# dakom/awsm-renderer

Hardware: AMD Instinct MI355X
Metric: frames/sec + shaded Mpix/s, 4K Sponza glTF, 1/2/4/8 MI355X (higher is better)
Workload: dtype f32; 1 GPU; Sponza-class procedural atrium (configs[3]): 262144 triangles, 25 materials, 69 textures, 3840x2160, geometry pass + opaque pass, single-sample, MipmapMode::None; triangles=262144, width=3840, height=2160, draws=92, frame_overlap=True, stream_handoff=device flags (k_handoff_signal / k_handoff_wait), camera=orbit, one turn per 240 frames, environment=uniform cubes (builder default), opaque_route=lean (k_shade_lean + k_shade_todo), library=awsm-renderer_amd/libawsm_hip.so

## Files before the change

### awsm-renderer_amd/csrc/device_math.hpp

```cpp
#pragma once
#include <hip/hip_runtime.h>
#include <hip/hip_fp16.h>
#include <stdint.h>

namespace awsm {

struct f2 { float x, y; };
struct f3 { float x, y, z; };
struct f4 { float x, y, z, w; };
struct m4 { f4 c[4]; };
struct m3 { f3 c[3]; };

#define AWSM_DI __device__ __forceinline__

constexpr float kPi = 3.1415926535897932384626433832795f;
constexpr float kTau = 6.283185307179586476925286766559f;
constexpr float kEps = 1e-4f;

AWSM_DI f2 mk2(float x, float y) { return {x, y}; }
AWSM_DI f3 mk3(float x, float y, float z) { return {x, y, z}; }
AWSM_DI f4 mk4(float x, float y, float z, float w) { return {x, y, z, w}; }
AWSM_DI f3 splat3(float s) { return {s, s, s}; }
AWSM_DI f3 operator+(f3 a, f3 b) { return {a.x + b.x, a.y + b.y, a.z + b.z}; }
AWSM_DI f3 operator-(f3 a, f3 b) { return {a.x - b.x, a.y - b.y, a.z - b.z}; }
AWSM_DI f3 operator*(f3 a, f3 b) { return {a.x * b.x, a.y * b.y, a.z * b.z}; }
AWSM_DI f3 operator*(f3 a, float s) { return {a.x * s, a.y * s, a.z * s}; }
AWSM_DI f3 operator/(f3 a, float s) { return {a.x / s, a.y / s, a.z / s}; }
AWSM_DI f3 operator-(f3 a) { return {-a.x, -a.y, -a.z}; }
AWSM_DI float dot(f3 a, f3 b) { return (a.x * b.x + a.y * b.y) + a.z * b.z; }
AWSM_DI f3 cross(f3 a, f3 b) { return {a.y * b.z - a.z * b.y, a.z * b.x - a.x * b.z, a.x * b.y - a.y * b.x}; }
AWSM_DI float length(f3 a) { return sqrtf(dot(a, a)); }
AWSM_DI f3 normalize(f3 a) { const float inv = 1.0f / length(a); return {a.x * inv, a.y * inv, a.z * inv}; }
AWSM_DI float mixf(float a, float b, float t) { return a * (1.0f - t) + b * t; }
AWSM_DI f3 mix3(f3 a, f3 b, float t) { float s = 1.0f - t; return {a.x * s + b.x * t, a.y * s + b.y * t, a.z * s + b.z * t}; }
AWSM_DI f3 min3(f3 a, f3 b) { return {fminf(a.x, b.x), fminf(a.y, b.y), fminf(a.z, b.z)}; }
AWSM_DI float clampf(float x, float lo, float hi) { return fminf(fmaxf(x, lo), hi); }
AWSM_DI float saturate(float x) { return clampf(x, 0.0f, 1.0f); }
AWSM_DI float inverse_sqrt(float x) { return 1.0f / sqrtf(x); }
AWSM_DI float signf(float x) { return x > 0.0f ? 1.0f : (x < 0.0f ? -1.0f : 0.0f); }

AWSM_DI f4 mul(const m4& m, f4 v) {
    f4 r;
    r.x = ((m.c[0].x * v.x + m.c[1].x * v.y) + m.c[2].x * v.z) + m.c[3].x * v.w;
    r.y = ((m.c[0].y * v.x + m.c[1].y * v.y) + m.c[2].y * v.z) + m.c[3].y * v.w;
    r.z = ((m.c[0].z * v.x + m.c[1].z * v.y) + m.c[2].z * v.z) + m.c[3].z * v.w;
    r.w = ((m.c[0].w * v.x + m.c[1].w * v.y) + m.c[2].w * v.z) + m.c[3].w * v.w;
    return r;
}
AWSM_DI f3 mul(const m3& m, f3 v) {
    f3 r;
    r.x = (m.c[0].x * v.x + m.c[1].x * v.y) + m.c[2].x * v.z;
    r.y = (m.c[0].y * v.x + m.c[1].y * v.y) + m.c[2].y * v.z;
    r.z = (m.c[0].z * v.x + m.c[1].z * v.y) + m.c[2].z * v.z;
    return r;
}
AWSM_DI m3 upper3(const m4& m) {
    m3 r;
    r.c[0] = {m.c[0].x, m.c[0].y, m.c[0].z};
    r.c[1] = {m.c[1].x, m.c[1].y, m.c[1].z};
    r.c[2] = {m.c[2].x, m.c[2].y, m.c[2].z};
    return r;
}
AWSM_DI m4 load_m4(const float* p) {
    const float4* q = reinterpret_cast<const float4*>(p);
    m4 m;
#pragma unroll
    for (int i = 0; i < 4; i++) { float4 v = q[i]; m.c[i] = {v.x, v.y, v.z, v.w}; }
    return m;
}

AWSM_DI float round_f16(float x) { return __half2float(__float2half_rn(x)); }
AWSM_DI unsigned short f16_bits(float x) { return __half_as_ushort(__float2half_rn(x)); }
AWSM_DI float f16_bits_to_f32(unsigned short h) { return __half2float(__ushort_as_half(h)); }

AWSM_DI float det_atan2f(float y, float x) {
    float ax = fabsf(x), ay = fabsf(y);
    float mx = fmaxf(ax, ay), mn = fminf(ax, ay);
    if (mx == 0.0f) return 0.0f;
    float a = mn / mx;
    float s = a * a;
    float r = 0.0027856871f;
    r = r * s - 0.0158660002f;
    r = r * s + 0.0424557589f;
    r = r * s - 0.0749753043f;
    r = r * s + 0.106448799f;
    r = r * s - 0.142070308f;
    r = r * s + 0.199934542f;
    r = r * s - 0.333331466f;
    r = r * s;
    r = r * a + a;
    if (ay > ax) r = 1.57079637f - r;
    if (x < 0.0f) r = 3.14159274f - r;
    if (y < 0.0f) r = -r;
    return r;
}

AWSM_DI f3 safe_normalize(f3 n) {
    float len_sq = dot(n, n);
    if (len_sq > 0.0f) return n * inverse_sqrt(len_sq);
    return {0.0f, 0.0f, 1.0f};
}
AWSM_DI float inverse_square(float range, float dist) {
    if (range == 0.0f) return 1.0f / fmaxf(dist * dist, 0.01f);
    float denom = dist * dist + 1.0f;
    float falloff = 1.0f - (dist * dist) / (range * range);
    return saturate(falloff * falloff) / denom;
}
AWSM_DI f2 encode_octahedral(f3 n_in) {
    const float inv = 1.0f / ((fabsf(n_in.x) + fabsf(n_in.y)) + fabsf(n_in.z));
    f3 n = {n_in.x * inv, n_in.y * inv, n_in.z * inv};
    if (n.z < 0.0f) {
        float wx = (1.0f - fabsf(n.y)) * signf(n.x);
        float wy = (1.0f - fabsf(n.x)) * signf(n.y);
        n.x = wx; n.y = wy;
    }
    return {n.x * 0.5f + 0.5f, n.y * 0.5f + 0.5f};
}
AWSM_DI f3 decode_octahedral(f2 e) {
    float fx = e.x * 2.0f - 1.0f, fy = e.y * 2.0f - 1.0f;
    f3 n = {fx, fy, (1.0f - fabsf(fx)) - fabsf(fy)};
    float t = clampf(-n.z, 0.0f, 1.0f);
    float vx = (n.x >= 0.0f) ? -t : t;
    float vy = (n.y >= 0.0f) ? -t : t;
    n = {n.x + vx, n.y + vy, n.z};
    return normalize(n);
}
struct TB { f3 t, b; };
AWSM_DI TB canonical_tb(f3 n) {
    TB r;
    if (n.z < -0.9999999f) {
        r.t = {0.0f, -1.0f, 0.0f};
        r.b = {-1.0f, 0.0f, 0.0f};
    } else {
        float a = 1.0f / (1.0f + n.z);
        float bb = (-n.x * n.y) * a;
        r.t = {1.0f - (n.x * n.x) * a, bb, -n.x};
        r.b = {bb, 1.0f - (n.y * n.y) * a, -n.y};
    }
    return r;
}
AWSM_DI f4 pack_normal_tangent(f3 N, f3 T, float s) {
    f2 oct = encode_octahedral(N);
    TB tb = canonical_tb(N);
    float x = dot(T, tb.t);
    float y = dot(T, tb.b);
    float theta = det_atan2f(y, x);
    float angle_u = (theta + kPi) / kTau;
    float sign_u = (s > 0.0f) ? 1.0f : 0.0f;
    return {oct.x, oct.y, angle_u, sign_u};
}
struct TBN { f3 N, T, B; };
AWSM_DI TBN unpack_normal_tangent(f4 rgba) {
    TBN r;
    r.N = decode_octahedral({rgba.x, rgba.y});
    float theta = rgba.z * kTau - kPi;
    float s = (rgba.w >= 0.5f) ? 1.0f : -1.0f;
    TB tb0 = canonical_tb(r.N);
    float c = cosf(theta), sn = sinf(theta);
    r.T = normalize(tb0.t * c + tb0.b * sn);
    r.B = normalize(cross(r.N, r.T)) * s;
    return r;
}

AWSM_DI float interp3_strict(float b0, float b1, float b2, float x0, float x1, float x2) { return (b0 * x0 + b1 * x1) + b2 * x2; }
AWSM_DI float affine2_strict(float a, float b, float c, float x, float y) { return (a * x + b * y) + c; }

AWSM_DI float blend_over_f16(float src, float dst, float one_minus_a) { return round_f16(src + dst * one_minus_a); }
AWSM_DI float resolve4_f16(float s0, float s1, float s2, float s3) { return round_f16((((s0 + s1) + s2) + s3) * 0.25f); }

}
```

### awsm-renderer_amd/csrc/kernels_shade.hip

```cpp
#include <type_traits>
#include "frame_params.hpp"
#include "raster_setup.hpp"

#ifndef AWSM_LEAN_WAVES
#define AWSM_LEAN_WAVES 6
#endif

namespace awsm {

struct GBufferTexel {
    f4 packed_nt;
    float bx, by;
    f4 bary_derivs;
};
template <bool DERIVS>
AWSM_DI GBufferTexel reconstruct_core(const TriSetup& t, float4 n0, float4 n1, float4 n2, float4 t0, float4 t1, float4 t2, int cx, int cy) {
    GBufferTexel g;
    g.bary_derivs = {0.0f, 0.0f, 0.0f, 0.0f};
    const double Xc = sample_coord((cx << 8) + 128), Yc = sample_coord((cy << 8) + 128);
    const EdgeVals ev = tri_edges_d(t, Xc, Yc);
    const float e0 = (float)ev.E[0] * t.iw[0], e1 = (float)ev.E[1] * t.iw[1], e2 = (float)ev.E[2] * t.iw[2];
    const float inv_esum = 1.0f / ((e0 + e1) + e2);
    const float b0 = e0 * inv_esum, b1 = e1 * inv_esum, b2 = e2 * inv_esum;
    const f3 Ni = {(b0 * n0.x + b1 * n1.x) + b2 * n2.x, (b0 * n0.y + b1 * n1.y) + b2 * n2.y, (b0 * n0.z + b1 * n1.z) + b2 * n2.z};
    const f4 Ti = {(b0 * t0.x + b1 * t1.x) + b2 * t2.x, (b0 * t0.y + b1 * t1.y) + b2 * t2.y,
                   (b0 * t0.z + b1 * t1.z) + b2 * t2.z, (b0 * t0.w + b1 * t1.w) + b2 * t2.w};
    const f4 p = pack_normal_tangent(normalize(Ni), normalize(mk3(Ti.x, Ti.y, Ti.z)), Ti.w);
    g.packed_nt = {round_f16(p.x), round_f16(p.y), round_f16(p.z), round_f16(p.w)};
    g.bx = round_f16(b0);
    g.by = round_f16(b1);
    if (DERIVS) {
        const EdgeVals eh = tri_edges_d(t, sample_coord(((cx ^ 1) << 8) + 128), Yc), evv = tri_edges_d(t, Xc, sample_coord(((cy ^ 1) << 8) + 128));
        const float h0 = (float)eh.E[0] * t.iw[0], h1 = (float)eh.E[1] * t.iw[1], h2 = (float)eh.E[2] * t.iw[2];
        const float w0 = (float)evv.E[0] * t.iw[0], w1 = (float)evv.E[1] * t.iw[1], w2 = (float)evv.E[2] * t.iw[2];
        const float ish = 1.0f / ((h0 + h1) + h2), isv = 1.0f / ((w0 + w1) + w2);
        const float hb0 = h0 * ish, hb1 = h1 * ish, vb0 = w0 * isv, vb1 = w1 * isv;
        const float ddx0 = (cx & 1) ? b0 - hb0 : hb0 - b0, ddx1 = (cx & 1) ? b1 - hb1 : hb1 - b1;
        const float ddy0 = (cy & 1) ? b0 - vb0 : vb0 - b0, ddy1 = (cy & 1) ? b1 - vb1 : vb1 - b1;
        g.bary_derivs = {round_f16(ddx0), round_f16(ddy0), round_f16(ddx1), round_f16(ddy1)};
    }
    return g;
}
template <bool DERIVS>
AWSM_DI GBufferTexel reconstruct_gbuffer(const FrameDev& f, uint32_t rank, int cx, int cy) {
    TriSetup t;
    tri_rec_load(f.tri_rec + rank, t);
    const float4 n0 = f.nrm[(size_t)rank * 3], n1 = f.nrm[(size_t)rank * 3 + 1], n2 = f.nrm[(size_t)rank * 3 + 2];
    const float4 t0 = f.tan[(size_t)rank * 3], t1 = f.tan[(size_t)rank * 3 + 1], t2 = f.tan[(size_t)rank * 3 + 2];
    return reconstruct_core<DERIVS>(t, n0, n1, n2, t0, t1, t2, cx, cy);
}

AWSM_DI f2 strict_oct_of(const FrameDev& f, uint32_t rank, int cx, int cy) {
    TriSetup t;
    tri_rec_load(f.tri_rec + rank, t);
    const float4 n0 = f.nrm[(size_t)rank * 3], n1 = f.nrm[(size_t)rank * 3 + 1], n2 = f.nrm[(size_t)rank * 3 + 2];
    const double Xc = sample_coord((cx << 8) + 128), Yc = sample_coord((cy << 8) + 128);
    const EdgeVals ev = tri_edges_d(t, Xc, Yc);
    const float e0 = (float)ev.E[0] * t.iw[0], e1 = (float)ev.E[1] * t.iw[1], e2 = (float)ev.E[2] * t.iw[2];
    const float inv_esum = 1.0f / ((e0 + e1) + e2);
    const float b0 = e0 * inv_esum, b1 = e1 * inv_esum, b2 = e2 * inv_esum;
    const f3 Ni = {(b0 * n0.x + b1 * n1.x) + b2 * n2.x, (b0 * n0.y + b1 * n1.y) + b2 * n2.y, (b0 * n0.z + b1 * n1.z) + b2 * n2.z};
    const f2 oct = encode_octahedral(normalize(Ni));
    return mk2(round_f16(oct.x), round_f16(oct.y));
}
AWSM_DI f3 strict_normal_of(const FrameDev& f, uint32_t rank, int cx, int cy) { return decode_octahedral(strict_oct_of(f, rank, cx, cy)); }
AWSM_DI uint32_t oct_word(f2 oct) { return (uint32_t)f16_bits(oct.x) | ((uint32_t)f16_bits(oct.y) << 16); }
AWSM_DI f2 oct_of_word(uint32_t w) { return mk2(__half2float(__ushort_as_half((unsigned short)(w & 0xFFFFu))), __half2float(__ushort_as_half((unsigned short)(w >> 16)))); }

AWSM_DI bool row_owned(const FrameDev& f, int py) {
    if (py < (int)f.sy0 || py >= (int)f.sy1) return false;
    return f.band_n <= 1u || (((uint32_t)py >> kTileShift) % f.band_n) == f.band_r;
}

constexpr float kEdgeNormalThreshold = 0.95f, kEdgeDepthThreshold = 0.02f, kEdgeMsaaDepthThreshold = 0.02f;
AWSM_DI float view_space_depth(const m4& inv_proj, float depth, float px, float py, float W, float H) {
    if (inv_proj.c[0].z == 0.0f && inv_proj.c[1].z == 0.0f && inv_proj.c[0].w == 0.0f && inv_proj.c[1].w == 0.0f)
        return (inv_proj.c[2].z * depth + inv_proj.c[3].z) / (inv_proj.c[2].w * depth + inv_proj.c[3].w);
    const f4 view_pos = mul(inv_proj, mk4((px / W) * 2.0f - 1.0f, 1.0f - (py / H) * 2.0f, depth, 1.0f));
    return view_pos.z / view_pos.w;
}
AWSM_DI float key_depth(unsigned long long k) { return k == ~0ull ? 1.0f : __uint_as_float((uint32_t)(k >> 32)); }
AWSM_DI uint32_t key_rank(unsigned long long k) { return 0xFFFFFFFFu - (uint32_t)(k & 0xFFFFFFFFull); }
AWSM_DI bool edge_mask_depth_msaa(const m4& inv_proj, const unsigned long long k4[4], float pcx, float pcy, float W, float H) {
    uint32_t count = 0; float dmin = 1e9f, dmax = -1e9f;
#pragma unroll
// ... 1780 lines not shown
                const m4 inv_proj = cload_m4(f.camera, 256u);
                const unsigned long long k4[4] = {((unsigned long long)ka.y << 32) | ka.x, ((unsigned long long)ka.w << 32) | ka.z, ((unsigned long long)kb.y << 32) | kb.x, ((unsigned long long)kb.w << 32) | kb.z};
                sure = edge_mask_depth_msaa_filtered(inv_proj, k4, (float)cx + 0.5f, (float)cy + 0.5f, (float)f.width, (float)f.height);
                test = !sure;
            }
        }
        const unsigned long long m_sure = __builtin_amdgcn_ballot_w64(sure), m_test = __builtin_amdgcn_ballot_w64(test);
        if (lane == 0u) *reinterpret_cast<ulonglong2*>(f.msaa_edge_bits + (size_t)(b.blk * 4u + (tid >> 6)) * 2u) = make_ulonglong2(m_sure, m_test);
        want_c0 = sure || test;
    }
    bool hud = false;
    if (!ITEMS && !MSAA && f.hud_vis && inside) { const u32x2 hk = gload<u32x2>(f.hud_vis, pv << 3); hud = (hk.x & hk.y) != 0xFFFFFFFFu; }
    if (hud) { store_pixel(f, p, f4{0.0f, 0.0f, 0.0f, 0.0f}); key = {0xFFFFFFFFu, 0xFFFFFFFFu}; }
    const bool hit = inside && (key.x & key.y) != 0xFFFFFFFFu;
    if (!ITEMS && inside && !hit && !hud) {
        const f4 sky = skybox_color(sc, f, cx, cy);
        store_pixel(f, p, sky);
        if (MSAA) {
            f.msaa_cells[pv] = make_uint2(0u, 0xFFFFFFFFu);
            if (want_c0) f.msaa_color0[pv] = make_float4(sky.x, sky.y, sky.z, sky.w);
        }
    }
    unsigned long long rem = __builtin_amdgcn_ballot_w64(hit);
    if (rem == 0ull) return true;
    const uint32_t rank = hit ? ~key.x : 0xFFFFFFFFu;
    const float depth = __uint_as_float(key.y);

    asm volatile("; MARK level1");
    unsigned long long src_base; uint32_t src_stride;
    {
        const uint32_t j = lane;
        const unsigned long long rec = (unsigned long long)f.tri_rec, nr = (unsigned long long)f.nrm, tn = (unsigned long long)f.tan, tsh = (unsigned long long)f.tri_shade;
        src_base = j < 5u ? rec + j * 16u : (j < 8u ? nr + (j - 5u) * 16u : (j < 11u ? tn + (j - 8u) * 16u : tsh + (j - 11u) * 16u));
        src_stride = j < 5u ? (uint32_t)kTriRecBytes : (j < 11u ? 48u : 32u);
    }
    uint32_t my_slot = kLeanNone, n_slots = 0u;
    while (rem != 0ull && n_slots < kLeanSlots) {
        const uint32_t r = (uint32_t)__builtin_amdgcn_readlane((int)rank, (int)__builtin_ctzll(rem));
        if (rank == r) my_slot = n_slots;
        if (lane < kLeanChunks)
            __builtin_amdgcn_global_load_lds((const AWSM_AS1 void*)(src_base + (unsigned long long)r * src_stride), (AWSM_AS3 void*)&st->q[n_slots][0], 16, 0, 0);
        rem &= ~__builtin_amdgcn_uicmp(rank, r, 32 );
        n_slots++;
    }
    asm volatile("s_waitcnt vmcnt(0)" ::: "memory");
    const bool staged = my_slot != kLeanNone;
    const uint4* rec = &st->q[staged ? my_slot : 0u][0];
    uint4 ts0 = rec[11], ts1 = rec[12];
    TriRecRaw raw;
    raw.q0 = bits_float4(rec[0]); raw.q1 = bits_float4(rec[1]); raw.q2 = bits_float4(rec[2]); raw.d3 = bits_double2(rec[3]); raw.d4 = bits_double2(rec[4]);
    float4 n0 = bits_float4(rec[5]), n1 = bits_float4(rec[6]), n2 = bits_float4(rec[7]);
    float4 t0 = bits_float4(rec[8]), t1 = bits_float4(rec[9]), t2 = bits_float4(rec[10]);
    if (hit && !staged) {
        ts0 = as_uint4(gload<u32x4>(f.tri_shade, rank << 5)); ts1 = as_uint4(gload<u32x4>(f.tri_shade, (rank << 5) + 16u));
        const uint32_t ro = rank * (uint32_t)kTriRecBytes, vo = rank * 48u;
        raw.q0 = as_float4(gload<f32x4>(f.tri_rec, ro)); raw.q1 = as_float4(gload<f32x4>(f.tri_rec, ro + 16u)); raw.q2 = as_float4(gload<f32x4>(f.tri_rec, ro + 32u));
        { const f64x2 a = gload<f64x2>(f.tri_rec, ro + 48u), c = gload<f64x2>(f.tri_rec, ro + 64u); raw.d3 = make_double2(a.x, a.y); raw.d4 = make_double2(c.x, c.y); }
        n0 = as_float4(gload<f32x4>(f.nrm, vo)); n1 = as_float4(gload<f32x4>(f.nrm, vo + 16u)); n2 = as_float4(gload<f32x4>(f.nrm, vo + 32u));
        t0 = as_float4(gload<f32x4>(f.tan, vo)); t1 = as_float4(gload<f32x4>(f.tan, vo + 16u)); t2 = as_float4(gload<f32x4>(f.tan, vo + 32u));
    }

    asm volatile("; MARK strict");
    TriSetup t;
    tri_rec_unpack(raw, t);
    const GBufferTexel g = reconstruct_core<(GRAD != 0)>(t, n0, n1, n2, t0, t1, t2, cx, cy);
    if (MSAA && hit) f.msaa_cells[pv] = make_uint2(oct_word(mk2(g.packed_nt.x, g.packed_nt.y)), key.y);
    const float bz = (1.0f - g.bx) - g.by;
    float u = interp3_strict(g.bx, g.by, bz, __uint_as_float(ts0.z), __uint_as_float(ts1.x), __uint_as_float(ts1.z));
    float v = interp3_strict(g.bx, g.by, bz, __uint_as_float(ts0.w), __uint_as_float(ts1.y), __uint_as_float(ts1.w));
    const uint32_t draw = ts0.x & 0x00FFFFFFu;
    const uint32_t d0 = (uint32_t)__builtin_amdgcn_readlane((int)draw, (int)__builtin_ctzll(__builtin_amdgcn_ballot_w64(hit)));
    const bool one_draw = __builtin_amdgcn_ballot_w64(hit && draw != d0) == 0ull;
    f2 ddx = {0.0f, 0.0f}, ddy = {0.0f, 0.0f};
    float m2 = 0.0f;
    float r2min = 0.0f; f2 major = {0.0f, 0.0f};
    if (GRAD) {
        const float x0 = __uint_as_float(ts0.z), y0 = __uint_as_float(ts0.w), x1 = __uint_as_float(ts1.x), y1 = __uint_as_float(ts1.y), x2 = __uint_as_float(ts1.z), y2 = __uint_as_float(ts1.w);
        const float dAlphaDx = g.bary_derivs.x, dAlphaDy = g.bary_derivs.y, dBetaDx = g.bary_derivs.z, dBetaDy = g.bary_derivs.w;
        const float dGammaDx = -dAlphaDx - dBetaDx, dGammaDy = -dAlphaDy - dBetaDy;
        ddx = {x0 * dAlphaDx + x1 * dBetaDx + x2 * dGammaDx, y0 * dAlphaDx + y1 * dBetaDx + y2 * dGammaDx};
        ddy = {x0 * dAlphaDy + x1 * dBetaDy + x2 * dGammaDy, y0 * dAlphaDy + y1 * dBetaDy + y2 * dGammaDy};
        const bool tiny = (fabsf(dAlphaDx) + fabsf(dAlphaDy) + fabsf(dBetaDx) + fabsf(dBetaDy)) < 1e-20f;
        const bool ok = (ddx.x == ddx.x) && (ddx.y == ddx.y) && (ddy.x == ddy.x) && (ddy.y == ddy.y);
        if (tiny || !ok) { ddx = {0.0f, 0.0f}; ddy = {0.0f, 0.0f}; }
    }
    if (GRAD == 0) {
    } else if (one_draw) {
        const uint32_t lo = d0 * (uint32_t)sizeof(LeanDrawDev);
        if (cload<uint32_t>(f.draw_lean, lo) & 8u) {
            const f32x4 ta = cload<f32x4>(f.draw_lean, lo + 176u); const f32x2a4 tb = cload<f32x2a4>(f.draw_lean, lo + 192u);
            const float u2 = affine2_strict(ta.x, ta.y, tb.x, u, v), v2 = affine2_strict(ta.z, ta.w, tb.y, u, v);
            u = u2; v = v2;
            if (GRAD) { ddx = {ta.x * ddx.x + ta.y * ddx.y, ta.z * ddx.x + ta.w * ddx.y}; ddy = {ta.x * ddy.x + ta.y * ddy.y, ta.z * ddy.x + ta.w * ddy.y}; }
        }
    } else {
// ... 17 lines not shown
    f3 base, emissive;
    float metallic_in, roughness_in, normal_scale, occlusion_strength, normal_bias, occlusion_bias;
    uint32_t exists;
    lean::Tap tp0, tp1, tp2, tp3, tp4;
    lean::TapG tg0, tg1, tg2, tg3, tg4;
    constexpr uint32_t kNeed = GRAD == 2 ? 7u : (GRAD ? 3u : 1u);
    auto fetch_all = [&](float uu, float vv, float m2e, bool act, const uint32_t tex_mask = 31u, const bool factors = true) {
        if (one_draw) {
            const uint32_t lo = d0 * (uint32_t)sizeof(LeanDrawDev);
            const u32x4 L0 = cload<u32x4>(f.draw_lean, lo), L1 = cload<u32x4>(f.draw_lean, lo + 16u), L2 = cload<u32x4>(f.draw_lean, lo + 32u);
            const u32x4 L3 = cload<u32x4>(f.draw_lean, lo + 48u), L4 = cload<u32x4>(f.draw_lean, lo + 64u);
            const u32x2 L5 = cload<u32x2>(f.draw_lean, lo + 80u), L5s = cload<u32x2>(f.draw_lean, lo + 88u);
            if (GRAD == 0) {
                if (L0.x & 8u) {
                    const f32x4 ta = cload<f32x4>(f.draw_lean, lo + 176u); const f32x2a4 tb = cload<f32x2a4>(f.draw_lean, lo + 192u);
                    const float u2 = affine2_strict(ta.x, ta.y, tb.x, uu, vv), v2 = affine2_strict(ta.z, ta.w, tb.y, uu, vv);
                    uu = u2; vv = v2;
                }
                todo = todo || __builtin_amdgcn_ballot_w64(hit && !(fabsf(uu) <= 32768.0f && fabsf(vv) <= 32768.0f)) != 0ull;
            }
            todo = todo || (L0.x & kNeed) != kNeed;
            const uint32_t exs = todo ? 0u : L0.x >> 8;
            const uint32_t ex = act ? exs & tex_mask : 0u;
            if (GRAD) {
                const u32x4 G0 = cload<u32x4>(f.draw_lean, lo + 96u), G1 = cload<u32x4>(f.draw_lean, lo + 112u), G2 = cload<u32x4>(f.draw_lean, lo + 128u);
                const u32x4 G3 = cload<u32x4>(f.draw_lean, lo + 144u), G4 = cload<u32x4>(f.draw_lean, lo + 160u);
                if (ex & 1u) lean::fetch_trilinear(lean::decode_g(G0.x, G0.y, G0.z, G0.w), m2e, uu, vv, tg0);
                if (ex & 2u) lean::fetch_trilinear(lean::decode_g(G1.x, G1.y, G1.z, G1.w), m2e, uu, vv, tg1);
                if (ex & 4u) lean::fetch_trilinear(lean::decode_g(G2.x, G2.y, G2.z, G2.w), m2e, uu, vv, tg2);
                if (ex & 8u) lean::fetch_trilinear(lean::decode_g(G3.x, G3.y, G3.z, G3.w), m2e, uu, vv, tg3);
                if (ex & 16u) lean::fetch_trilinear(lean::decode_g(G4.x, G4.y, G4.z, G4.w), m2e, uu, vv, tg4);
            } else {
                if (ex & 1u) lean::fetch_s(lean::decode_s(L3.x, L3.y), uu, vv, tp0);
                if (ex & 2u) lean::fetch_s(lean::decode_s(L3.z, L3.w), uu, vv, tp1);
                if (ex & 4u) lean::fetch_s(lean::decode_s(L4.x, L4.y), uu, vv, tp2);
                if (ex & 8u) lean::fetch_s(lean::decode_s(L4.z, L4.w), uu, vv, tp3);
                if (ex & 16u) lean::fetch_s(lean::decode_s(L5.x, L5.y), uu, vv, tp4);
            }
            exists = exs;
            if (factors) {
            metallic_in = __uint_as_float(L0.y); roughness_in = __uint_as_float(L0.z); normal_scale = __uint_as_float(L0.w);
            base = {__uint_as_float(L1.x), __uint_as_float(L1.y), __uint_as_float(L1.z)}; occlusion_strength = __uint_as_float(L1.w);
            emissive = {__uint_as_float(L2.x), __uint_as_float(L2.y), __uint_as_float(L2.z)}; normal_bias = __uint_as_float(L2.w); occlusion_bias = __uint_as_float(L5s.x);
            }
        } else {
            const uint32_t lo = draw * (uint32_t)sizeof(LeanDrawDev);
// ... 52 lines not shown
    auto mid = [&]() {
    asm volatile("; MARK standard");
    const float pxf = (float)cx, pyf = (float)cy;
    const float* M = f.pix2view;
    const float hx = M[0] * pxf + (M[4] * pyf + (M[8] * depth + M[12])), hy = M[1] * pxf + (M[5] * pyf + (M[9] * depth + M[13]));
    const float hz = M[2] * pxf + (M[6] * pyf + (M[10] * depth + M[14])), hw = M[3] * pxf + (M[7] * pyf + (M[11] * depth + M[15]));
    const float ivw = fm::rcp(fmaxf(hw, 1e-8f));
    const f3 vp = {hx * ivw, hy * ivw, hz * ivw};
    const float* R = f.view_rot;
    const f3 rel = {R[0] * vp.x + (R[3] * vp.y + R[6] * vp.z), R[1] * vp.x + (R[4] * vp.y + R[7] * vp.z), R[2] * vp.x + (R[5] * vp.y + R[8] * vp.z)};
    world_position = {rel.x + f.cam_pos[0], rel.y + f.cam_pos[1], rel.z + f.cam_pos[2]};
#ifdef AWSM_STRICT_POSITION
    world_position = strict_world_position(cload_m4(f.camera, 256u), cload_m4(f.camera, 320u), cx, cy, (float)f.width, (float)f.height, depth);
#endif
    if (f.cam_ortho) {
        surface_to_camera = mk3(f.ortho_view_dir[0], f.ortho_view_dir[1], f.ortho_view_dir[2]);
    } else {
        const f3 to_camera = mk3(f.cam_pos[0], f.cam_pos[1], f.cam_pos[2]) - world_position;
        surface_to_camera = fm::fdot(to_camera, to_camera) > 0.0f ? fm::fsafe_normalize(to_camera) : mk3(0.0f, 0.0f, 1.0f);
    }
    asm volatile("; MARK tbn");
    tbn = fm::funpack_normal_tangent(g.packed_nt);
    normal = tbn.N;
    };
    bool shared_fp = false;
    float Lm = 0.0f;
    auto lean_word = [&](auto one, uint32_t off) {
        if constexpr (decltype(one)::value) return cload<uint32_t>(f.draw_lean, d0 * (uint32_t)sizeof(LeanDrawDev) + off);
        else return gload<uint32_t>(f.draw_lean, draw * (uint32_t)sizeof(LeanDrawDev) + off);
    };
    auto lean_quad = [&](auto one, uint32_t off) {
        if constexpr (decltype(one)::value) return cload<u32x4>(f.draw_lean, d0 * (uint32_t)sizeof(LeanDrawDev) + off);
        else return gload<u32x4>(f.draw_lean, draw * (uint32_t)sizeof(LeanDrawDev) + off);
    };
    auto decide = [&](auto one) {
        const uint32_t fl = lean_word(one, 0u);
        const uint32_t exs = (fl & kNeed) == kNeed ? (fl >> 8) & 31u : 0u;
        int lw_min = 15, top_min = 15;
#pragma unroll
        for (uint32_t k = 0; k < (uint32_t)kCoreTextures; k++) {
            const uint32_t w1 = lean_word(one, 96u + 16u * k + 4u);
            const int lw = (int)(w1 >> 24), lv = (int)((w1 >> 16) & 15u);
            if (exs & (1u << k)) { lw_min = min(lw_min, lw); top_min = min(top_min, lv - 1 - lw); }
        }
        Lm = 0.5f * __builtin_amdgcn_logf(fmaxf(m2c, 1e-30f));
        const bool in = exs != 0u && Lm > -(float)lw_min && Lm < (float)top_min;
// ... 192 lines not shown
    for (uint32_t i = 0; i < n_lights; i++) {
        const f32x4 pre0 = cload<f32x4>(f.lights_pre, i * 32u), pre1 = cload<f32x4>(f.lights_pre, i * 32u + 16u);
        const uint32_t kind = (uint32_t)pre0.w;
        f3 light_dir = {pre0.x, pre0.y, pre0.z}, radiance = {pre1.x, pre1.y, pre1.z};
        if (kind == 2u || kind == 3u) {
            const f32x4 pos_range = cload<f32x4>(lights, i * 64u);
            const f3 stl = mk3(pos_range.x, pos_range.y, pos_range.z) - world_position;
            const float d2 = fm::fdot(stl, stl);
            const float inv_d = d2 > 0.0f ? fm::rsq(d2) : 0.0f;
            const float dist = d2 * inv_d;
            float att;
            if (pos_range.w == 0.0f) att = fm::rcp(fmaxf(dist * dist, 0.01f));
            else { const float fo = 1.0f - fm::fdiv(dist * dist, pos_range.w * pos_range.w); att = fm::fdiv(saturate(fo * fo), dist * dist + 1.0f); }
            const f3 to_light = stl * inv_d;
            if (kind == 3u) {
                const f32x4 dir_inner = cload<f32x4>(lights, i * 64u + 16u), kind_outer = cload<f32x4>(lights, i * 64u + 48u);
                const float cos_l = fm::fdot(to_light, -light_dir);
                const float sm = saturate(fm::fdiv(cos_l - kind_outer.y, dir_inner.w - kind_outer.y));
                att = att * (sm * sm);
            }
            light_dir = to_light;
            radiance = radiance * att;
#ifndef AWSM_NO_LIGHT_SKIP
            if (__builtin_amdgcn_ballot_w64(!(att == 0.0f)) == 0ull) continue;
#endif
        } else if (kind != 1u) { light_dir = {0.0f, 0.0f, 0.0f}; radiance = {0.0f, 0.0f, 0.0f}; }
        lean::direct(lit, light_dir, radiance, color);
    }
    asm volatile("; MARK store");
    if (ITEMS) { item->color = color; return true; }
    store_pixel(f, p, {color.x, color.y, color.z, 1.0f});
    if (MSAA && want_c0) f.msaa_color0[pv] = make_float4(color.x, color.y, color.z, 1.0f);
    return true;
}
template <int GRAD, bool MSAA>
AWSM_DI void lean_block(const DevScene* __restrict__ sc, const FrameDev& f, const ShadeBlock& b, const uint32_t wg, const uint32_t tid, LeanStage* __restrict__ st) {
    (void)lean_core<GRAD, MSAA, false>(sc, f, b, wg, tid, st, nullptr);
}
#ifndef AWSM_ANISO_WAVES
#define AWSM_ANISO_WAVES 4
#endif
#ifndef AWSM_LEAN_COUNTERS
#define AWSM_LEAN_COUNTERS 8
#endif
constexpr uint32_t kLeanCounters = AWSM_LEAN_COUNTERS;
#ifndef AWSM_LEAN_GRAD_WAVES
#define AWSM_LEAN_GRAD_WAVES 5
#endif
template <bool PERSIST, int GRAD, bool MSAA>
// ... 11 lines not shown
    const uint32_t w = __builtin_amdgcn_readfirstlane((blockIdx.x >> 3) * 4u + (threadIdx.x >> 6));
    uint32_t zero;
    asm volatile("v_mov_b32 %0, 0" : "=v"(zero));
    uint32_t c = w % kLeanCounters, tried = 0u;
    uint32_t* ctr0 = f.lean_next + (xcd * kLeanCounters) * 16u + zero;
    uint32_t nxt = 0u;
    if (PERSIST && lane == 0u) nxt = atomicAdd(ctr0 + c * 16u, 1u);
    for (uint32_t j = w;;) {
        if (PERSIST) {
            j = __builtin_amdgcn_readfirstlane(nxt) * kLeanCounters + c;
            while (j >= share && ++tried < kLeanCounters) {
                c = (c + 1u) % kLeanCounters;
                if (lane == 0u) nxt = atomicAdd(ctr0 + c * 16u, 1u);
                j = __builtin_amdgcn_readfirstlane(nxt) * kLeanCounters + c;
            }
            if (j >= share) break;
            if (lane == 0u) nxt = atomicAdd(ctr0 + c * 16u, 1u);
        }
        const uint32_t kb = j >> 2, bcol = kb & ((1u << lp) - 1u), brow = (kb >> lp) * 8u + xcd;
        if (bcol < bx_n && j < share) {
            ShadeBlock b;
            shade_block_at(f, b, brow, bcol);
            lean_block<GRAD, MSAA>(sc, f, b, ((kb >> lp) * bx_n + bcol) * 8u + xcd, ((j & 3u) << 6) | lane, st);
        }
        if (!PERSIST) break;
    }
}

constexpr uint32_t kEdgeRecBytes = 260;
struct NeighbourCell { float nx, ny, nz; uint32_t depth_bits; uint32_t state; };

AWSM_DI void publish_cell(NeighbourCell* cells, int lx, int ly, const FrameDev& f, int px, int py) {
    NeighbourCell c = {0.0f, 0.0f, 0.0f, 0u, 0u};
    if (px >= 0 && px < (int)f.width && py >= (int)f.y0 && py < (int)f.y1) {
        unsigned long long k;
        if (f.band_n > 1u && (((uint32_t)py >> kTileShift) % f.band_n) != f.band_r) {
            const uint32_t ty = (uint32_t)py >> kTileShift, which = ((uint32_t)py & (uint32_t)(kTile - 1)) == 0u ? 0u : 1u;
            k = f.msaa_halo ? f.msaa_halo[((((size_t)(ty % f.band_n) * f.halo_bands + ty / f.band_n) * 2u + which) * f.width) + (size_t)px] : ~0ull;
        } else k = f.vis[((size_t)py * f.width + (size_t)px) * 4];
        c.state = 1u;
        if (k != ~0ull) {
            const f3 n = strict_normal_of(f, key_rank(k), px, py);
            c.nx = n.x; c.ny = n.y; c.nz = n.z; c.depth_bits = (uint32_t)(k >> 32); c.state = 2u;
        }
    }
    cells[(ly + 1) * 18 + (lx + 1)] = c;
}
// ... 403 lines not shown
    const DrawDev dr = draws[tri_info[rank] & 0x00FFFFFFu];
    const uint32_t material_meta_offset = *reinterpret_cast<const uint32_t*>(sc->buf[AWSM_BUF_GEOM_META] + dr.geom_meta_off + 36);
    const uint32_t* mm = reinterpret_cast<const uint32_t*>(sc->buf[AWSM_BUF_MATERIAL_META] + (size_t)(material_meta_offset / 256u) * 256u);
    out[0] = 1u; out[1] = mm[0]; out[2] = mm[1]; out[3] = rank - dr.first_tri;
}

__global__ void k_rgba16f_to_rg16f(const uint16_t* __restrict__ in, uint32_t* __restrict__ out, uint32_t n) {
    const uint32_t i = blockIdx.x * 256u + threadIdx.x;
    if (i < n) out[i] = (uint32_t)in[(size_t)i * 4] | ((uint32_t)in[(size_t)i * 4 + 1] << 16);
}

}

extern "C" void awsm_launch_resolve_draws(const awsm::DevScene* sc, const awsm::FrameDev* f, hipStream_t s) {
    if (f->n_draws) hipLaunchKernelGGL(awsm::k_resolve_draws, dim3((8u * f->n_draws + 255u) / 256u), dim3(256), 0, s, sc, *f);
}
#define AWSM_LAUNCH_G(g, K, grid, block, ...) do { if ((g) == 2) hipLaunchKernelGGL((K<2>), grid, block, 0, s, __VA_ARGS__); else if ((g) == 1) hipLaunchKernelGGL((K<1>), grid, block, 0, s, __VA_ARGS__); \
                                                   else hipLaunchKernelGGL((K<0>), grid, block, 0, s, __VA_ARGS__); } while (0)
#define AWSM_LAUNCH_G2(g, K, B, grid, block, ...) do { if ((g) == 2) hipLaunchKernelGGL((K<2, B>), grid, block, 0, s, __VA_ARGS__); else if ((g) == 1) hipLaunchKernelGGL((K<1, B>), grid, block, 0, s, __VA_ARGS__); \
                                                       else hipLaunchKernelGGL((K<0, B>), grid, block, 0, s, __VA_ARGS__); } while (0)
#define AWSM_LAUNCH_SG(g, K, S, grid, block, ...) do { if ((g) == 2) hipLaunchKernelGGL((K<S, 2>), grid, block, 0, s, __VA_ARGS__); else if ((g) == 1) hipLaunchKernelGGL((K<S, 1>), grid, block, 0, s, __VA_ARGS__); \
                                                       else hipLaunchKernelGGL((K<S, 0>), grid, block, 0, s, __VA_ARGS__); } while (0)
static inline int mip_mode(const awsm::FrameDev* f) { return f->mipmap ? (f->aniso ? 2 : 1) : 0; }
extern "C" int awsm_shade_is_lean(const awsm::FrameDev* f);
extern "C" void awsm_launch_shade(const awsm::DevScene* sc, const awsm::FrameDev* f, hipStream_t s) {
    const uint32_t bx_n = (f->width + 15u) >> 4, by_n = f->band_n > 1u ? 2u * f->tiles_y : ((f->sy1 - f->sy0) + 15u) >> 4;
    const uint32_t nb = 8u * ((by_n + 7u) / 8u) * bx_n;
    if (!nb) return;
    const int g = mip_mode(f);
    const bool msaa = f->msaa == 4u;
    if (awsm_shade_is_lean(f)) {
        uint32_t pitch = 1; while (pitch < bx_n) pitch <<= 1;
        const uint32_t nb_ids = 8u * ((by_n + 7u) / 8u) * pitch;
        if (msaa) {
            if (g == 2) hipLaunchKernelGGL((awsm::k_shade_lean<false, 2, true>), dim3(nb_ids), dim3(256), 0, s, sc, *f);
            else if (g == 1) hipLaunchKernelGGL((awsm::k_shade_lean<false, 1, true>), dim3(nb_ids), dim3(256), 0, s, sc, *f);
            else hipLaunchKernelGGL((awsm::k_shade_lean<false, 0, true>), dim3(nb_ids), dim3(256), 0, s, sc, *f);
        } else if (g == 2) hipLaunchKernelGGL((awsm::k_shade_lean<false, 2, false>), dim3(nb_ids), dim3(256), 0, s, sc, *f);
        else if (g == 1) hipLaunchKernelGGL((awsm::k_shade_lean<false, 1, false>), dim3(nb_ids), dim3(256), 0, s, sc, *f);
        else if (f->lean_grid && f->lean_next) hipLaunchKernelGGL((awsm::k_shade_lean<true, 0, false>), dim3(min(f->lean_grid, nb_ids)), dim3(256), 0, s, sc, *f);
        else hipLaunchKernelGGL((awsm::k_shade_lean<false, 0, false>), dim3(nb_ids), dim3(256), 0, s, sc, *f);
        return;
    }
    if (msaa) {
        AWSM_LAUNCH_G(g, awsm::k_shade_msaa, dim3(nb), dim3(256), sc, *f);
        AWSM_LAUNCH_G(g, awsm::k_shade_msaa_resolve, dim3(nb), dim3(64), sc, *f);
// ... 57 lines not shown
```

Measured before the change: 3437 frames/s.

## Use fast rcp/sqrt with range tracking and plain fallback in G-buffer reconstruction

Replaces IEEE-correct f32 division, reciprocal and sqrt in normal/tangent reconstruction with a hardware rcp/sqrt plus Newton refinement sequence. Each lane tracks the operand exponent range, and if any lane in the wave falls outside the safe range the whole reconstruction is recomputed with the plain operators. It also adds wave-level debug counters, compiled only under debug macros. The aim is to avoid the long scaling and fixup sequences of correctly rounded division, at the cost of extra range bookkeeping and a possible redo on rare waves.

Result: no change. 3425 frames/s, median of 2 (-0.4%).

```diff
diff --git a/awsm-renderer_amd/csrc/device_math.hpp b/awsm-renderer_amd/csrc/device_math.hpp
--- a/awsm-renderer_amd/csrc/device_math.hpp
+++ b/awsm-renderer_amd/csrc/device_math.hpp
@@ -16,6 +16,76 @@
 constexpr float kPi = 3.1415926535897932384626433832795f;
 constexpr float kTau = 6.283185307179586476925286766559f;
 constexpr float kEps = 1e-4f;
+
+constexpr uint32_t kStrictLoBits = 0x29000000u;
+constexpr uint32_t kStrictHiBits = 0x56000000u;
+#define AWSM_HDI __host__ __device__ __forceinline__
+AWSM_HDI float strict_div_core(float a, float b) {
+#if defined(__HIP_DEVICE_COMPILE__)
+    float r = __builtin_amdgcn_rcpf(b);
+    const float e = __builtin_fmaf(-b, r, 1.0f);
+    r = __builtin_fmaf(e, r, r);
+    float q = a * r;
+    const float e1 = __builtin_fmaf(-b, q, a);
+    q = __builtin_fmaf(e1, r, q);
+    const float e2 = __builtin_fmaf(-b, q, a);
+    return __builtin_fmaf(e2, r, q);
+#else
+    return a / b;
+#endif
+}
+AWSM_HDI float strict_sqrt_core(float x) {
+#if defined(__HIP_DEVICE_COMPILE__)
+    float s = __builtin_amdgcn_sqrtf(x);
+    const float sd = __builtin_bit_cast(float, __builtin_bit_cast(uint32_t, s) - 1u), su = __builtin_bit_cast(float, __builtin_bit_cast(uint32_t, s) + 1u);
+    const float rd = __builtin_fmaf(-sd, s, x), ru = __builtin_fmaf(-su, s, x);
+    s = (0.0f >= rd) ? sd : s;
+    s = (0.0f < ru) ? su : s;
+    return s;
+#else
+    return sqrtf(x);
+#endif
+}
+AWSM_HDI bool strict_in_range(float x) { const uint32_t u = __builtin_bit_cast(uint32_t, x) & 0x7FFFFFFFu; return u >= kStrictLoBits && u <= kStrictHiBits; }
+AWSM_HDI bool strict_div_in_range(float a, float b) { return strict_in_range(b) && (strict_in_range(a) || __builtin_bit_cast(uint32_t, a) == 0u); }
+AWSM_HDI bool strict_sqrt_in_range(float x) { const uint32_t u = __builtin_bit_cast(uint32_t, x); return u >= kStrictLoBits && u <= kStrictHiBits; }
+AWSM_HDI float strict_div(float a, float b) {
+#if defined(__HIP_DEVICE_COMPILE__)
+    if (__builtin_amdgcn_ballot_w64(!strict_div_in_range(a, b)) == 0ull) return strict_div_core(a, b);
+#endif
+    return a / b;
+}
+AWSM_HDI float strict_rcp(float x) {
+#if defined(__HIP_DEVICE_COMPILE__)
+    if (__builtin_amdgcn_ballot_w64(!strict_in_range(x)) == 0ull) return strict_div_core(1.0f, x);
+#endif
+    return 1.0f / x;
+}
+AWSM_HDI float strict_sqrt(float x) {
+#if defined(__HIP_DEVICE_COMPILE__)
+    if (__builtin_amdgcn_ballot_w64(!strict_sqrt_in_range(x)) == 0ull) return strict_sqrt_core(x);
+#endif
+    return sqrtf(x);
+}
+struct StrictPlain {
+    AWSM_HDI float div(float a, float b) { return a / b; }
+    AWSM_HDI float div_bounded(float a, float b) { return a / b; }
+    AWSM_HDI float rcp(float x) { return 1.0f / x; }
+    AWSM_HDI float rcp_bounded(float x) { return 1.0f / x; }
+    AWSM_HDI float sqrt(float x) { return sqrtf(x); }
+    AWSM_HDI bool ok() const { return true; }
+};
+struct StrictFast {
+    uint32_t lo = 0xFFFFFFFFu, hi = 0u, nlo = 0xFFFFFFFFu;
+    AWSM_HDI void den(float x) { const uint32_t u = __builtin_bit_cast(uint32_t, x) & 0x7FFFFFFFu; lo = u < lo ? u : lo; hi = u > hi ? u : hi; }
+    AWSM_HDI void num(float a) { const uint32_t u = __builtin_bit_cast(uint32_t, a); nlo = u - 1u < nlo ? u - 1u : nlo; hi = u > hi ? u : hi; }
+    AWSM_HDI float div(float a, float b) { num(a); den(b); return strict_div_core(a, b); }
+    AWSM_HDI float div_bounded(float a, float b) { return strict_div_core(a, b); }
+    AWSM_HDI float rcp(float x) { den(x); return strict_div_core(1.0f, x); }
+    AWSM_HDI float rcp_bounded(float x) { return strict_div_core(1.0f, x); }
+    AWSM_HDI float sqrt(float x) { const uint32_t u = __builtin_bit_cast(uint32_t, x); lo = u < lo ? u : lo; hi = u > hi ? u : hi; return strict_sqrt_core(x); }
+    AWSM_HDI bool ok() const { return lo >= kStrictLoBits && hi <= kStrictHiBits && nlo >= kStrictLoBits - 1u; }
+};
 
 AWSM_DI f2 mk2(float x, float y) { return {x, y}; }
 AWSM_DI f3 mk3(float x, float y, float z) { return {x, y, z}; }
@@ -30,7 +100,8 @@
 AWSM_DI float dot(f3 a, f3 b) { return (a.x * b.x + a.y * b.y) + a.z * b.z; }
 AWSM_DI f3 cross(f3 a, f3 b) { return {a.y * b.z - a.z * b.y, a.z * b.x - a.x * b.z, a.x * b.y - a.y * b.x}; }
 AWSM_DI float length(f3 a) { return sqrtf(dot(a, a)); }
-AWSM_DI f3 normalize(f3 a) { const float inv = 1.0f / length(a); return {a.x * inv, a.y * inv, a.z * inv}; }
+template <class M> AWSM_DI f3 normalize(f3 a, M& m) { const float inv = m.rcp_bounded(m.sqrt(dot(a, a))); return {a.x * inv, a.y * inv, a.z * inv}; }
+AWSM_DI f3 normalize(f3 a) { StrictPlain m; return normalize(a, m); }
 AWSM_DI float mixf(float a, float b, float t) { return a * (1.0f - t) + b * t; }
 AWSM_DI f3 mix3(f3 a, f3 b, float t) { float s = 1.0f - t; return {a.x * s + b.x * t, a.y * s + b.y * t, a.z * s + b.z * t}; }
 AWSM_DI f3 min3(f3 a, f3 b) { return {fminf(a.x, b.x), fminf(a.y, b.y), fminf(a.z, b.z)}; }
@@ -73,11 +144,11 @@
 AWSM_DI unsigned short f16_bits(float x) { return __half_as_ushort(__float2half_rn(x)); }
 AWSM_DI float f16_bits_to_f32(unsigned short h) { return __half2float(__ushort_as_half(h)); }
 
-AWSM_DI float det_atan2f(float y, float x) {
+template <class M> AWSM_DI float det_atan2f(float y, float x, M& m) {
     float ax = fabsf(x), ay = fabsf(y);
     float mx = fmaxf(ax, ay), mn = fminf(ax, ay);
     if (mx == 0.0f) return 0.0f;
-    float a = mn / mx;
+    float a = m.div(mn, mx);
     float s = a * a;
     float r = 0.0027856871f;
     r = r * s - 0.0158660002f;
@@ -94,6 +165,7 @@
     if (y < 0.0f) r = -r;
     return r;
 }
+AWSM_DI float det_atan2f(float y, float x) { StrictPlain m; return det_atan2f(y, x, m); }
 
 AWSM_DI f3 safe_normalize(f3 n) {
     float len_sq = dot(n, n);
@@ -106,8 +178,8 @@
     float falloff = 1.0f - (dist * dist) / (range * range);
     return saturate(falloff * falloff) / denom;
 }
-AWSM_DI f2 encode_octahedral(f3 n_in) {
-    const float inv = 1.0f / ((fabsf(n_in.x) + fabsf(n_in.y)) + fabsf(n_in.z));
+template <class M> AWSM_DI f2 encode_octahedral(f3 n_in, M& m) {
+    const float inv = m.rcp((fabsf(n_in.x) + fabsf(n_in.y)) + fabsf(n_in.z));
     f3 n = {n_in.x * inv, n_in.y * inv, n_in.z * inv};
     if (n.z < 0.0f) {
         float wx = (1.0f - fabsf(n.y)) * signf(n.x);
@@ -116,6 +188,7 @@
     }
     return {n.x * 0.5f + 0.5f, n.y * 0.5f + 0.5f};
 }
+AWSM_DI f2 encode_octahedral(f3 n_in) { StrictPlain m; return encode_octahedral(n_in, m); }
 AWSM_DI f3 decode_octahedral(f2 e) {
     float fx = e.x * 2.0f - 1.0f, fy = e.y * 2.0f - 1.0f;
     f3 n = {fx, fy, (1.0f - fabsf(fx)) - fabsf(fy)};
@@ -126,29 +199,31 @@
     return normalize(n);
 }
 struct TB { f3 t, b; };
-AWSM_DI TB canonical_tb(f3 n) {
+template <class M> AWSM_DI TB canonical_tb(f3 n, M& m) {
     TB r;
     if (n.z < -0.9999999f) {
         r.t = {0.0f, -1.0f, 0.0f};
         r.b = {-1.0f, 0.0f, 0.0f};
     } else {
-        float a = 1.0f / (1.0f + n.z);
+        float a = m.rcp(1.0f + n.z);
         float bb = (-n.x * n.y) * a;
         r.t = {1.0f - (n.x * n.x) * a, bb, -n.x};
         r.b = {bb, 1.0f - (n.y * n.y) * a, -n.y};
     }
     return r;
 }
-AWSM_DI f4 pack_normal_tangent(f3 N, f3 T, float s) {
-    f2 oct = encode_octahedral(N);
-    TB tb = canonical_tb(N);
+AWSM_DI TB canonical_tb(f3 n) { StrictPlain m; return canonical_tb(n, m); }
+template <class M> AWSM_DI f4 pack_normal_tangent(f3 N, f3 T, float s, M& m) {
+    f2 oct = encode_octahedral(N, m);
+    TB tb = canonical_tb(N, m);
     float x = dot(T, tb.t);
     float y = dot(T, tb.b);
-    float theta = det_atan2f(y, x);
-    float angle_u = (theta + kPi) / kTau;
+    float theta = det_atan2f(y, x, m);
+    float angle_u = m.div(theta + kPi, kTau);
     float sign_u = (s > 0.0f) ? 1.0f : 0.0f;
     return {oct.x, oct.y, angle_u, sign_u};
 }
+AWSM_DI f4 pack_normal_tangent(f3 N, f3 T, float s) { StrictPlain m; return pack_normal_tangent(N, T, s, m); }
 struct TBN { f3 N, T, B; };
 AWSM_DI TBN unpack_normal_tangent(f4 rgba) {
     TBN r;
diff --git a/awsm-renderer_amd/csrc/kernels_shade.hip b/awsm-renderer_amd/csrc/kernels_shade.hip
--- a/awsm-renderer_amd/csrc/kernels_shade.hip
+++ b/awsm-renderer_amd/csrc/kernels_shade.hip
@@ -7,25 +7,35 @@
 #endif
 
 namespace awsm {
+
+enum : uint32_t { kCntWaves = 0, kCntNoHit, kCntSlotTrips, kCntUnstaged, kCntOneDraw, kCntMultiDraw, kCntTextures, kCntLightsEntered, kCntLightsSkipped,
+                  kCntLightsOther, kCntTodo, kCntStrictRedo, kCntPadding, kCntTbnStrict, kCntLeanCounters };
+#if defined(AWSM_DEBUG_SWITCHES) && defined(AWSM_LEAN_COUNTERS)
+__device__ unsigned int g_lean_counters[kCntLeanCounters];
+#define AWSM_COUNT_N(i, n) do { if ((threadIdx.x & 63u) == (uint32_t)__builtin_ctzll(__builtin_amdgcn_ballot_w64(true))) atomicAdd(&g_lean_counters[i], (unsigned int)(n)); } while (0)
+#else
+#define AWSM_COUNT_N(i, n) do { } while (0)
+#endif
+#define AWSM_COUNT(i) AWSM_COUNT_N(i, 1u)
 
 struct GBufferTexel {
     f4 packed_nt;
     float bx, by;
     f4 bary_derivs;
 };
-template <bool DERIVS>
-AWSM_DI GBufferTexel reconstruct_core(const TriSetup& t, float4 n0, float4 n1, float4 n2, float4 t0, float4 t1, float4 t2, int cx, int cy) {
+template <bool DERIVS, class M>
+AWSM_DI GBufferTexel reconstruct_core_on(M& m, const TriSetup& t, float4 n0, float4 n1, float4 n2, float4 t0, float4 t1, float4 t2, int cx, int cy) {
     GBufferTexel g;
     g.bary_derivs = {0.0f, 0.0f, 0.0f, 0.0f};
     const double Xc = sample_coord((cx << 8) + 128), Yc = sample_coord((cy << 8) + 128);
     const EdgeVals ev = tri_edges_d(t, Xc, Yc);
     const float e0 = (float)ev.E[0] * t.iw[0], e1 = (float)ev.E[1] * t.iw[1], e2 = (float)ev.E[2] * t.iw[2];
-    const float inv_esum = 1.0f / ((e0 + e1) + e2);
+    const float inv_esum = m.rcp((e0 + e1) + e2);
     const float b0 = e0 * inv_esum, b1 = e1 * inv_esum, b2 = e2 * inv_esum;
     const f3 Ni = {(b0 * n0.x + b1 * n1.x) + b2 * n2.x, (b0 * n0.y + b1 * n1.y) + b2 * n2.y, (b0 * n0.z + b1 * n1.z) + b2 * n2.z};
     const f4 Ti = {(b0 * t0.x + b1 * t1.x) + b2 * t2.x, (b0 * t0.y + b1 * t1.y) + b2 * t2.y,
                    (b0 * t0.z + b1 * t1.z) + b2 * t2.z, (b0 * t0.w + b1 * t1.w) + b2 * t2.w};
-    const f4 p = pack_normal_tangent(normalize(Ni), normalize(mk3(Ti.x, Ti.y, Ti.z)), Ti.w);
+    const f4 p = pack_normal_tangent(normalize(Ni, m), normalize(mk3(Ti.x, Ti.y, Ti.z), m), Ti.w, m);
     g.packed_nt = {round_f16(p.x), round_f16(p.y), round_f16(p.z), round_f16(p.w)};
     g.bx = round_f16(b0);
     g.by = round_f16(b1);
@@ -33,11 +43,22 @@
         const EdgeVals eh = tri_edges_d(t, sample_coord(((cx ^ 1) << 8) + 128), Yc), evv = tri_edges_d(t, Xc, sample_coord(((cy ^ 1) << 8) + 128));
         const float h0 = (float)eh.E[0] * t.iw[0], h1 = (float)eh.E[1] * t.iw[1], h2 = (float)eh.E[2] * t.iw[2];
         const float w0 = (float)evv.E[0] * t.iw[0], w1 = (float)evv.E[1] * t.iw[1], w2 = (float)evv.E[2] * t.iw[2];
-        const float ish = 1.0f / ((h0 + h1) + h2), isv = 1.0f / ((w0 + w1) + w2);
+        const float ish = m.rcp((h0 + h1) + h2), isv = m.rcp((w0 + w1) + w2);
         const float hb0 = h0 * ish, hb1 = h1 * ish, vb0 = w0 * isv, vb1 = w1 * isv;
         const float ddx0 = (cx & 1) ? b0 - hb0 : hb0 - b0, ddx1 = (cx & 1) ? b1 - hb1 : hb1 - b1;
         const float ddy0 = (cy & 1) ? b0 - vb0 : vb0 - b0, ddy1 = (cy & 1) ? b1 - vb1 : vb1 - b1;
         g.bary_derivs = {round_f16(ddx0), round_f16(ddy0), round_f16(ddx1), round_f16(ddy1)};
+    }
+    return g;
+}
+template <bool DERIVS>
+AWSM_DI GBufferTexel reconstruct_core(const TriSetup& t, float4 n0, float4 n1, float4 n2, float4 t0, float4 t1, float4 t2, int cx, int cy, bool live = true) {
+    StrictFast fast;
+    GBufferTexel g = reconstruct_core_on<DERIVS>(fast, t, n0, n1, n2, t0, t1, t2, cx, cy);
+    if (__builtin_expect(__builtin_amdgcn_ballot_w64(live && !fast.ok()) != 0ull, 0)) {
+        AWSM_COUNT(kCntStrictRedo);
+        StrictPlain plain;
+        g = reconstruct_core_on<DERIVS>(plain, t, n0, n1, n2, t0, t1, t2, cx, cy);
     }
     return g;
 }
@@ -57,10 +78,15 @@
     const double Xc = sample_coord((cx << 8) + 128), Yc = sample_coord((cy << 8) + 128);
     const EdgeVals ev = tri_edges_d(t, Xc, Yc);
     const float e0 = (float)ev.E[0] * t.iw[0], e1 = (float)ev.E[1] * t.iw[1], e2 = (float)ev.E[2] * t.iw[2];
-    const float inv_esum = 1.0f / ((e0 + e1) + e2);
-    const float b0 = e0 * inv_esum, b1 = e1 * inv_esum, b2 = e2 * inv_esum;
-    const f3 Ni = {(b0 * n0.x + b1 * n1.x) + b2 * n2.x, (b0 * n0.y + b1 * n1.y) + b2 * n2.y, (b0 * n0.z + b1 * n1.z) + b2 * n2.z};
-    const f2 oct = encode_octahedral(normalize(Ni));
+    auto on = [&](auto& m) {
+        const float inv_esum = m.rcp((e0 + e1) + e2);
+        const float b0 = e0 * inv_esum, b1 = e1 * inv_esum, b2 = e2 * inv_esum;
+        const f3 Ni = {(b0 * n0.x + b1 * n1.x) + b2 * n2.x, (b0 * n0.y + b1 * n1.y) + b2 * n2.y, (b0 * n0.z + b1 * n1.z) + b2 * n2.z};
+        return encode_octahedral(normalize(Ni, m), m);
+    };
+    StrictFast fast;
+    f2 oct = on(fast);
+    if (__builtin_expect(__builtin_amdgcn_ballot_w64(!fast.ok()) != 0ull, 0)) { StrictPlain plain; oct = on(plain); }
     return mk2(round_f16(oct.x), round_f16(oct.y));
 }
 AWSM_DI f3 strict_normal_of(const FrameDev& f, uint32_t rank, int cx, int cy) { return decode_octahedral(strict_oct_of(f, rank, cx, cy)); }
@@ -1887,7 +1913,8 @@
         }
     }
     unsigned long long rem = __builtin_amdgcn_ballot_w64(hit);
-    if (rem == 0ull) return true;
+    if (!ITEMS) AWSM_COUNT(kCntWaves);
+    if (rem == 0ull) { if (!ITEMS) AWSM_COUNT(kCntNoHit); return true; }
     const uint32_t rank = hit ? ~key.x : 0xFFFFFFFFu;
     const float depth = __uint_as_float(key.y);
 
@@ -1910,6 +1937,7 @@
     }
     asm volatile("s_waitcnt vmcnt(0)" ::: "memory");
     const bool staged = my_slot != kLeanNone;
+    if (!ITEMS) { AWSM_COUNT_N(kCntSlotTrips, n_slots); if (__builtin_amdgcn_ballot_w64(hit && !staged) != 0ull) AWSM_COUNT(kCntUnstaged); }
     const uint4* rec = &st->q[staged ? my_slot : 0u][0];
     uint4 ts0 = rec[11], ts1 = rec[12];
     TriRecRaw raw;
@@ -1928,7 +1956,7 @@
     asm volatile("; MARK strict");
     TriSetup t;
     tri_rec_unpack(raw, t);
-    const GBufferTexel g = reconstruct_core<(GRAD != 0)>(t, n0, n1, n2, t0, t1, t2, cx, cy);
+    const GBufferTexel g = reconstruct_core<(GRAD != 0)>(t, n0, n1, n2, t0, t1, t2, cx, cy, hit);
     if (MSAA && hit) f.msaa_cells[pv] = make_uint2(oct_word(mk2(g.packed_nt.x, g.packed_nt.y)), key.y);
     const float bz = (1.0f - g.bx) - g.by;
     float u = interp3_strict(g.bx, g.by, bz, __uint_as_float(ts0.z), __uint_as_float(ts1.x), __uint_as_float(ts1.z));
@@ -1936,6 +1964,7 @@
     const uint32_t draw = ts0.x & 0x00FFFFFFu;
     const uint32_t d0 = (uint32_t)__builtin_amdgcn_readlane((int)draw, (int)__builtin_ctzll(__builtin_amdgcn_ballot_w64(hit)));
     const bool one_draw = __builtin_amdgcn_ballot_w64(hit && draw != d0) == 0ull;
+    if (!ITEMS) AWSM_COUNT(one_draw ? kCntOneDraw : kCntMultiDraw);
     f2 ddx = {0.0f, 0.0f}, ddy = {0.0f, 0.0f};
     float m2 = 0.0f;
     float r2min = 0.0f; f2 major = {0.0f, 0.0f};
@@ -1999,6 +2028,7 @@
             todo = todo || (L0.x & kNeed) != kNeed;
             const uint32_t exs = todo ? 0u : L0.x >> 8;
             const uint32_t ex = act ? exs & tex_mask : 0u;
+            if (!ITEMS) AWSM_COUNT_N(kCntTextures, __builtin_popcount(exs & tex_mask));
             if (GRAD) {
                 const u32x4 G0 = cload<u32x4>(f.draw_lean, lo + 96u), G1 = cload<u32x4>(f.draw_lean, lo + 112u), G2 = cload<u32x4>(f.draw_lean, lo + 128u);
                 const u32x4 G3 = cload<u32x4>(f.draw_lean, lo + 144u), G4 = cload<u32x4>(f.draw_lean, lo + 160u);
@@ -2097,6 +2127,7 @@
     asm volatile("; MARK tbn");
     tbn = fm::funpack_normal_tangent(g.packed_nt);
     normal = tbn.N;
+    if (!ITEMS && __builtin_amdgcn_ballot_w64(hit && tbn.N.z < -0.98f) != 0ull) AWSM_COUNT(kCntTbnStrict);
     };
     bool shared_fp = false;
     float Lm = 0.0f;
@@ -2335,9 +2366,10 @@
             light_dir = to_light;
             radiance = radiance * att;
 #ifndef AWSM_NO_LIGHT_SKIP
-            if (__builtin_amdgcn_ballot_w64(!(att == 0.0f)) == 0ull) continue;
+            if (__builtin_amdgcn_ballot_w64(!(att == 0.0f)) == 0ull) { if (!ITEMS) AWSM_COUNT(kCntLightsSkipped); continue; }
 #endif
-        } else if (kind != 1u) { light_dir = {0.0f, 0.0f, 0.0f}; radiance = {0.0f, 0.0f, 0.0f}; }
+            if (!ITEMS) AWSM_COUNT(kCntLightsEntered);
+        } else { if (!ITEMS) AWSM_COUNT(kCntLightsOther); if (kind != 1u) { light_dir = {0.0f, 0.0f, 0.0f}; radiance = {0.0f, 0.0f, 0.0f}; } }
         lean::direct(lit, light_dir, radiance, color);
     }
     asm volatile("; MARK store");
@@ -2395,7 +2427,7 @@
             ShadeBlock b;
             shade_block_at(f, b, brow, bcol);
             lean_block<GRAD, MSAA>(sc, f, b, ((kb >> lp) * bx_n + bcol) * 8u + xcd, ((j & 3u) << 6) | lane, st);
-        }
+        } else AWSM_COUNT(kCntPadding);
         if (!PERSIST) break;
     }
 }
@@ -2845,6 +2877,13 @@
 #define AWSM_LAUNCH_SG(g, K, S, grid, block, ...) do { if ((g) == 2) hipLaunchKernelGGL((K<S, 2>), grid, block, 0, s, __VA_ARGS__); else if ((g) == 1) hipLaunchKernelGGL((K<S, 1>), grid, block, 0, s, __VA_ARGS__); \
                                                        else hipLaunchKernelGGL((K<S, 0>), grid, block, 0, s, __VA_ARGS__); } while (0)
 static inline int mip_mode(const awsm::FrameDev* f) { return f->mipmap ? (f->aniso ? 2 : 1) : 0; }
+#if defined(AWSM_DEBUG_SWITCHES) && defined(AWSM_LEAN_COUNTERS)
+extern "C" int awsm_debug_lean_counters(unsigned int* out, int clear) {
+    if (out && hipMemcpyFromSymbol(out, HIP_SYMBOL(awsm::g_lean_counters), sizeof(unsigned int) * awsm::kCntLeanCounters) != hipSuccess) return -1;
+    if (clear) { const unsigned int z[awsm::kCntLeanCounters] = {}; if (hipMemcpyToSymbol(HIP_SYMBOL(awsm::g_lean_counters), z, sizeof(z)) != hipSuccess) return -1; }
+    return (int)awsm::kCntLeanCounters;
+}
+#endif
 extern "C" int awsm_shade_is_lean(const awsm::FrameDev* f);
 extern "C" void awsm_launch_shade(const awsm::DevScene* sc, const awsm::FrameDev* f, hipStream_t s) {
     const uint32_t bx_n = (f->width + 15u) >> 4, by_n = f->band_n > 1u ? 2u * f->tiles_y : ((f->sy1 - f->sy0) + 15u) >> 4;
```
